# elliottower/gobblet-rl

Measured on AMD Instinct MI355X. Metric: env-steps/sec at 2^20 parallel boards, 1/2/4/8 MI355X; bit-exact mask/winner, higher is better.
Workload: dtype int8

## Files before the change

### gobblet-rl_amd/csrc/gobblet_hip.hip

```cpp
#include "gobblet_device.h"

#include <stdio.h>
#include <algorithm>
#include <type_traits>
#include <utility>
#include <stdlib.h>
#include <string.h>

#include "../../include/gobblet_hip.h"
#include "gobblet_diag.h"
#include "gobblet_knobs.h"

using namespace gbl;

namespace {

thread_local char g_err[256] = "";

int fail(int code, const char *msg)
{
    snprintf(g_err, sizeof g_err, "%s", msg);
    return code;
}

// ... 830 lines not shown
        }
        if (A.first_actions && t == 0) {
            action = given;
            if (SC)
                y = play_ply<false, PAIR>(p, row, mover, legal, action, A.illegal_mode, j);
            else
                y = play_ply<false, PAIR>(p, NoRow{}, mover, legal, action, A.illegal_mode, j);
        } else {
            if (SC)
                y = play_ply<true, PAIR>(p, row, mover, legal, action, A.illegal_mode, j);
            else
                y = play_ply<true, PAIR>(p, NoRow{}, mover, legal, action, A.illegal_mode, j);
        }
        GBL_PHASE_DEP(2, (uint32_t)y.winner + p.nz);
        dn = y.terminal ? 1 : 0;
        uint64_t legal_next = legal54(p, mover);
        if (y.terminal) {
            p = Planes{0u, 0u, 0u};
            mover = 0;
            legal_next = kLegalEmpty;
            if (SC) row.reset();
        }
        GBL_PHASE_DEP(3, p.nz);
        if (t) {
            if constexpr (OB) sub_store<kObs, kRowPolicy, BPS>(odst, vo, lane, obytes & ~15);
            if constexpr (MK) sub_store<kActions, kRowPolicy, BPS>(mdst, vm, lane, mbytes & ~15);
        }
        if constexpr (SC) {
            tcount = next_turn(tcount, y, 1);
            treset = treset || y.terminal;
            if (A.counters) {
                games += __popcll(__ballot(valid && j == 0 && y.terminal));
                w1 += __popcll(__ballot(valid && j == 0 && y.winner == 1));
                w2 += __popcll(__ballot(valid && j == 0 && y.winner == -1));
            }
            {
                const uint16_t rw = (uint16_t)((y.r0 & 0xFF) | ((y.r1 & 0xFF) << 8));
                if (sc_act) sc_act[at] = action;
                if (sc_rw) sc_rw[at] = rw;
                if (sc_b0) sc_b0[at] = (int8_t)(LPB == 1 ? y.winner : b0_is_mover ? mover : b0_is_winner ? y.winner : dn);
                if constexpr (LPB <= 2) {
                    if (sc_b1) sc_b1[at] = (int8_t)(LPB == 1 ? dn : y.winner);
                }
                if constexpr (LPB == 1) {
                    if (sc_b2) sc_b2[at] = (int8_t)mover;
                }
                at += A.ply_stride;
            }
        }
        GBL_PHASE(4);
        if constexpr (OB) {
            sub_obs_zero<BPS>(obs_img, lane);
            wave_lds_fence();
            obs_scatter_part<LPB>(reinterpret_cast<uint8_t *>(obs_img) + bq * kObs, p, mover, j);
            wave_lds_fence();
            odst = obs_at;
            obs_at += obs_step;
            sub_fetch<kObs, BPS>(obs_img, lane, vo);
            if (!full) sub_tail(odst, obs_img, lane, obytes);
            wave_lds_fence();
        }
        GBL_PHASE(5);
        legal = legal_next;
        GBL_PHASE_DEP(6, (uint32_t)legal);
        if constexpr (MK) {
            mask_row_part<LPB>(reinterpret_cast<uint8_t *>(mask_img) + bq * kActions, legal, j);
            wave_lds_fence();
            mdst = mask_at;
            mask_at += mask_step;
            sub_fetch<kActions, BPS>(mask_img, lane, vm);
            if (!full) sub_tail(mdst, mask_img, lane, mbytes);
            wave_lds_fence();
        }
        GBL_PHASE(7);
    }
    GBL_PHASE(7);
    GBL_PHASE_FLUSH(wave_index());
    if (plies) {
        if constexpr (OB) sub_store<kObs, kRowPolicy, BPS>(odst, vo, lane, obytes & ~15);
        if constexpr (MK) sub_store<kActions, kRowPolicy, BPS>(mdst, vm, lane, mbytes & ~15);
    }
    if constexpr (SC) {
        wave_lds_fence();
        sub_out<kCells, kStorePlain, BPS>(A.state + sub * (BPS * kCells), img, lane, rows);
        if (valid && j == 0) {
            A.to_move[b] = (int8_t)mover;
            A.done[b] = (int8_t)dn;
            if (A.turn) A.turn[b] = treset ? tcount : A.turn[b] + tcount;
        }
        if (A.counters && lane == 0) tally_flush(A.counters, sub >> SH, rows, plies, games, w1, w2);
    }
}

template <bool WITH_MASK, bool WITH_OBS, bool DEV_PLY, bool HAND>
__global__ __launch_bounds__(64 * (1 + (WITH_MASK ? 1 : 0) + (WITH_OBS ? 1 : 0))) void k_collect3(
    int8_t *__restrict__ state, int8_t *__restrict__ to_move, int64_t n, int64_t ntiles, uint64_t seed, uint64_t env_base,
    const uint32_t *__restrict__ ply_dev, uint32_t ply0, uint32_t plies, int8_t *__restrict__ done, int64_t ply_stride,
    int64_t tile_stride, int32_t *__restrict__ actions_t, int8_t *__restrict__ winner_t, int8_t *__restrict__ reward_t,
    int8_t *__restrict__ done_t, int8_t *__restrict__ to_move_t, int8_t *__restrict__ mask_t, int8_t *__restrict__ obs_t,
    int illegal_mode, int64_t *__restrict__ counters, int32_t *__restrict__ turn, const int32_t *__restrict__ first_actions,
    int8_t *__restrict__ first_status)
{
    constexpr int WAVES = 1 + (WITH_MASK ? 1 : 0) + (WITH_OBS ? 1 : 0);
    __shared__ uint32_t s_state[image_words<kCells>()];
    __shared__ uint32_t s_obs[WITH_OBS ? image_words<kObs>() : 4];
    __shared__ uint32_t s_mask[WITH_MASK ? image_words<kActions>() : 4];
    __shared__ uint4 s_hand[2][kTile];
    using LegalSlot = typename std::conditional<HAND, uint4, uint2>::type;
    __shared__ LegalSlot s_legal[2][kTile];
    if (DEV_PLY) ply0 += *ply_dev;
    const int role = WAVES > 1 ? wave_index() : 0;
    const int lane = (int)(threadIdx.x & 63u);
    const int64_t tile = (int64_t)blockIdx.x;
    if (tile >= ntiles) return;
    const int64_t left = n - tile * kTile;
    const int rows = left < kTile ? (int)left : kTile;
    const bool valid = lane < rows, full = rows == kTile;
    const int64_t b = tile * kTile + lane;
    constexpr int kPolicy = kStoreStreamDrop;
    const int64_t cell0 = tile * tile_stride;
    constexpr bool hand_scalars = HAND && WAVES > 1;
    if (role != 0) {
        const bool is_mask = WITH_MASK && role == 1;
        SubVecs<WITH_MASK ? sub_vectors<kActions, kTile>() : 0> vm{};
        SubVecs<WITH_OBS ? sub_vectors<kObs, kTile>() : 0> vo{};
        int8_t *dst = nullptr;
        int8_t *row_at = is_mask ? mask_t + cell0 * kActions : obs_t + cell0 * kObs;
        const int64_t row_step = ply_stride * (is_mask ? kActions : kObs);
        int64_t scell = cell0 + lane;
        for (uint32_t t = 0; t < plies; ++t) {
            pair_barrier();
            if constexpr (hand_scalars) {
                if (role == 1) {
                    const uint4 sc = s_legal[t & 1u][lane];
                    if (valid) {
                        if (actions_t) actions_t[scell] = (int32_t)sc.z;
                        if (winner_t) winner_t[scell] = (int8_t)(sc.w & 0xFFu);
                        if (reward_t) reinterpret_cast<uint16_t *>(reward_t)[scell] = (uint16_t)((sc.w >> 8) & 0xFFFFu);
                        if (done_t) done_t[scell] = (int8_t)((sc.w >> 24) & 1u);
                        if (to_move_t) to_move_t[scell] = (int8_t)((sc.w >> 25) & 1u);
                    }
                    scell += ply_stride;
                }
            }
            if (t) {
                if constexpr (WITH_MASK) {
                    if (is_mask) sub_store<kActions, kPolicy, kTile>(dst, vm, lane, (rows * kActions) & ~15);
                }
                if constexpr (WITH_OBS) {
                    if (!is_mask) sub_store<kObs, kPolicy, kTile>(dst, vo, lane, (rows * kObs) & ~15);
                }
            }
            if constexpr (WITH_MASK) {
                if (is_mask) {
                    const LegalSlot lg = s_legal[t & 1u][lane];
                    mask_row_part<1>(reinterpret_cast<uint8_t *>(s_mask) + lane * kActions, ((uint64_t)lg.y << 32) | lg.x, 0);
                    wave_lds_fence();
                    dst = row_at;
                    sub_fetch<kActions, kTile>(s_mask, lane, vm);
                    if (!full) sub_tail(dst, s_mask, lane, rows * kActions);
                    wave_lds_fence();
                }
            }
            if constexpr (WITH_OBS) {
                if (!is_mask) {
                    const uint4 h = s_hand[t & 1u][lane];
                    sub_obs_zero<kTile>(s_obs, lane);
                    wave_lds_fence();
                    obs_scatter_row(reinterpret_cast<uint8_t *>(s_obs) + lane * kObs, Planes{h.x, h.y, h.z}, (int)h.w);
                    wave_lds_fence();
                    dst = row_at;
                    sub_fetch<kObs, kTile>(s_obs, lane, vo);
                    if (!full) sub_tail(dst, s_obs, lane, rows * kObs);
                    wave_lds_fence();
                }
            }
            row_at += row_step;
        }
        if (plies) {
            if constexpr (WITH_MASK) {
                if (is_mask) sub_store<kActions, kPolicy, kTile>(dst, vm, lane, (rows * kActions) & ~15);
            }
            if constexpr (WITH_OBS) {
                if (!is_mask) sub_store<kObs, kPolicy, kTile>(dst, vo, lane, (rows * kObs) & ~15);
            }
        }
        return;
    }
    Lane L;
    L.tile = tile; L.lane = lane; L.rows = rows; L.valid = valid; L.b = b;
    int mover = to_move[valid ? b : n - 1];
    int given = first_actions ? first_actions[valid ? b : n - 1] : 0;
    uint32_t r[7];
    Draw4 block{{0u, 0u, 0u, 0u}};
    load_state(state, s_state, L, r, [&] { block = draw_block(seed, env_base + (uint64_t)b, ply0); });
    mover = valid && mover != 0;
    Planes p = planes_of(L, r);
    const ImageRow row{reinterpret_cast<uint8_t *>(s_state) + lane * kCells};
    uint32_t games = 0, w1 = 0, w2 = 0;
    Ply y{0, 0, 0, false, false};
    int dn = 0, tcount = 0;
    bool treset = false;
    uint64_t legal = legal54(p, mover);
    if (first_status && valid) first_status[b] = (int8_t)action_status_of(legal, given);
    int64_t cell = cell0;
    for (uint32_t t = 0; t < plies; ++t) {
        const uint32_t ply = ply0 + t;
        int action = pick54(legal, draw_word(block, ply));
        if (t + 1 < plies && ((ply + 1) & 3u) == 0) block = draw_block(seed, env_base + (uint64_t)b, ply + 1);
        if (first_actions && t == 0) {
            action = given;
            y = play_ply(p, row, mover, legal, action, illegal_mode);
        } else {
            y = play_ply<true>(p, row, mover, legal, action, illegal_mode);
        }
        dn = y.terminal ? 1 : 0;
        legal = legal54(p, mover);
        if (y.terminal) {
            p = Planes{0u, 0u, 0u};
            mover = 0;
            legal = kLegalEmpty;
            row.reset();
        }
        s_hand[t & 1u][lane] = uint4{p.nz, p.neg, p.odd, (uint32_t)mover};
        if constexpr (HAND)
            s_legal[t & 1u][lane] = uint4{(uint32_t)legal, (uint32_t)(legal >> 32), (uint32_t)action,
                                          ((uint32_t)y.winner & 0xFFu) | (((uint32_t)y.r0 & 0xFFu) << 8) | (((uint32_t)y.r1 & 0xFFu) << 16) |
                                              ((uint32_t)dn << 24) | ((uint32_t)mover << 25)};
        else
            s_legal[t & 1u][lane] = uint2{(uint32_t)legal, (uint32_t)(legal >> 32)};
        if (WAVES > 1) pair_barrier();
        tcount = next_turn(tcount, y, 1);
        treset = treset || y.terminal;
        if (counters) {
            games += __popcll(__ballot(valid && y.terminal));
            w1 += __popcll(__ballot(valid && y.winner == 1));
            w2 += __popcll(__ballot(valid && y.winner == -1));
        }
        if (!hand_scalars && valid) {
            const int64_t at = cell + lane;
            if (actions_t) actions_t[at] = action;
            if (winner_t) winner_t[at] = (int8_t)y.winner;
            if (reward_t) reinterpret_cast<uint16_t *>(reward_t)[at] = (uint16_t)((y.r0 & 0xFF) | ((y.r1 & 0xFF) << 8));
            if (done_t) done_t[at] = (int8_t)dn;
            if (to_move_t) to_move_t[at] = (int8_t)mover;
        }
        cell += ply_stride;
    }
    wave_lds_fence();
    tile_out<kCells>(state + tile * (kTile * kCells), s_state, lane, rows);
    if (valid) {
        to_move[b] = (int8_t)mover;
        done[b] = (int8_t)dn;
        if (turn) turn[b] = treset ? tcount : turn[b] + tcount;
    }
    if (counters && lane == 0) tally_flush(counters, tile, rows, plies, games, w1, w2);
}

template <bool WITH_MASK, bool WITH_OBS, int KO, bool MERGE>
constexpr int small_waves() { return 1 + ((WITH_MASK && !MERGE) ? 1 : 0) + (WITH_OBS ? KO : 0); }

template <bool WITH_MASK, bool WITH_OBS, bool DEV_PLY, int LA, int KO, bool MERGE>
__global__ __launch_bounds__((64 * small_waves<WITH_MASK, WITH_OBS, KO, MERGE>())) void k_collect_small(
    int8_t *__restrict__ state, int8_t *__restrict__ to_move, int64_t n, int64_t ngroups, uint64_t seed, uint64_t env_base,
    const uint32_t *__restrict__ ply_dev, uint32_t ply0, uint32_t plies, int8_t *__restrict__ done, int64_t ply_stride,
    int64_t tile_stride, int32_t *__restrict__ actions_t, int8_t *__restrict__ winner_t, int8_t *__restrict__ reward_t,
    int8_t *__restrict__ done_t, int8_t *__restrict__ to_move_t, int8_t *__restrict__ mask_t, int8_t *__restrict__ obs_t,
    int illegal_mode, int64_t *__restrict__ counters, int32_t *__restrict__ turn, const int32_t *__restrict__ first_actions,
    int8_t *__restrict__ first_status)
{
    static_assert(LA * KO <= 4 && (KO > 0 || MERGE), "at most four lanes per board");
    constexpr int WAVES = small_waves<WITH_MASK, WITH_OBS, KO, MERGE>(), NA = WAVES - (WITH_OBS ? KO : 0);
    constexpr int GB = kTile / LA, LO = LA * (KO ? KO : 1), OBB = kTile / LO;
    constexpr int kStateWords = GB * kCells / 4 + 4, kObsWords = OBB * kObs / 4 + 4, kMaskWords = GB * kActions / 4 + 4;
    __shared__ uint32_t s_state[WAVES][kStateWords];
    __shared__ uint32_t s_obs[WITH_OBS && KO ? KO : 1][WITH_OBS ? kObsWords : 4];
    __shared__ uint32_t s_mask[WITH_MASK ? kMaskWords : 4];
    __shared__ uint4 s_draw[LO > 1 ? WAVES : 1][LO > 1 ? 64 : 1];
    if (DEV_PLY) ply0 += *ply_dev;
    const int64_t group = (int64_t)blockIdx.x;
    if (group >= ngroups) return;
    const int wave = WAVES > 1 ? wave_index() : 0;
    const SmallArgs A{state, to_move, done, n, seed, env_base, ply0, plies, ply_stride, tile_stride, actions_t, winner_t, reward_t,
                      done_t, to_move_t, mask_t, obs_t, illegal_mode, counters, turn, first_actions, first_status};
    constexpr bool SYNC = WAVES > 1;
    if (wave == 0) {
        small_role<kRoleScalars | ((WITH_MASK && MERGE) ? kRoleMask : 0) | ((WITH_OBS && KO == 0) ? kRoleObs : 0), LA, SYNC>(
            A, s_state[0], s_mask, s_obs[0], reinterpret_cast<uint32_t *>(s_draw[0]), group);
        return;
    }
    if constexpr (WITH_MASK && !MERGE) {
        if (wave == 1) {
            small_role<kRoleMask, LA, SYNC>(A, s_state[1], s_mask, nullptr, reinterpret_cast<uint32_t *>(s_draw[LO > 1 ? 1 : 0]), group);
            return;
        }
    }
    if constexpr (WITH_OBS && KO > 0)
        small_role<kRoleObs, LO, SYNC>(A, s_state[wave], nullptr, s_obs[wave - NA], reinterpret_cast<uint32_t *>(s_draw[LO > 1 ? wave : 0]),
                                       group * KO + (wave - NA));
}

constexpr int kGroupBoards = 32, kGroupRing = 4;

template <bool WITH_OBS, bool DEV_PLY>
__global__ __launch_bounds__(64 * (WITH_OBS ? 4 : 2)) void k_collect5(
    int8_t *__restrict__ state, int8_t *__restrict__ to_move, int64_t n, int64_t ngroups, uint64_t seed, uint64_t env_base,
    const uint32_t *__restrict__ ply_dev, uint32_t ply0, uint32_t plies, int8_t *__restrict__ done, int64_t ply_stride,
    int64_t tile_stride, int32_t *__restrict__ actions_t, int8_t *__restrict__ winner_t, int8_t *__restrict__ reward_t,
    int8_t *__restrict__ done_t, int8_t *__restrict__ to_move_t, int8_t *__restrict__ mask_t, int8_t *__restrict__ obs_t,
    int illegal_mode, int64_t *__restrict__ counters, int32_t *__restrict__ turn, const int32_t *__restrict__ first_actions,
    int8_t *__restrict__ first_status)
{
    constexpr int GB = kGroupBoards, OBB = 16;
    static_assert(kGroupRing == 4, "slot = t & 7, one generator block per group of plies");
    __shared__ uint32_t s_state[GB * kCells / 4 + 4];
    __shared__ uint32_t s_mask[GB * kActions / 4 + 4];
    __shared__ uint32_t s_obs[WITH_OBS ? 2 : 1][WITH_OBS ? OBB * kObs / 4 + 4 : 4];
    __shared__ uint4 s_hand[2 * kGroupRing][GB];
    __shared__ uint4 s_legal[2 * kGroupRing][GB];
    __shared__ uint4 s_draw[4][GB];
    if (DEV_PLY) ply0 += *ply_dev;
    const int role = wave_index();
    const int lane = (int)(threadIdx.x & 63u);
    const int64_t group = (int64_t)blockIdx.x;
    if (group >= ngroups) return;
    const int64_t left = n - group * GB;
    const int rows = left < GB ? (int)left : GB;
    constexpr int kPolicy = kStoreStreamDrop;
    const int64_t cell0 = (group >> 1) * tile_stride + (group & 1) * GB;
    const uint32_t m0 = ply0 >> 2;
    const uint32_t groups_of_plies = (plies + kGroupRing - 1) / kGroupRing;
    if (role == 1) {
        const int bq = lane >> 1, j = lane & 1;
        const bool valid = bq < rows;
        const int64_t b = group * GB + bq;
        SubVecs<sub_vectors<kActions, GB>()> vm{};
        int8_t *dst = nullptr, *row_at = mask_t + cell0 * kActions;
        const int64_t row_step = ply_stride * kActions;
        const int mbytes = rows * kActions;
        int32_t *sc_act = nullptr;
        uint16_t *sc_rw = nullptr;
        int8_t *sc_b0 = nullptr, *sc_b1 = nullptr;
        if (valid) {
            const int64_t at0 = cell0 + bq;
            if (j == 0 && actions_t) sc_act = actions_t + at0;
            if (j == 1 && reward_t) sc_rw = reinterpret_cast<uint16_t *>(reward_t) + at0;
            int8_t *const arr = j == 0 ? to_move_t : done_t;
            if (arr) sc_b0 = arr + at0;
            if (j == 0 && winner_t) sc_b1 = winner_t + at0;
        }
        int64_t at = 0;
        uint32_t games = 0, w1 = 0, w2 = 0;
        int tcount = 0;
        bool treset = false;
        auto generate = [&](uint32_t m) {
            const Draw4 d = draw_block(seed, env_base + (uint64_t)b, m << 2);
            s_draw[m & 3u][bq] = uint4{d.w[0], d.w[1], d.w[2], d.w[3]};
        };
        generate(m0);
        generate(m0 + 1u);
        generate(m0 + 2u);
        pair_barrier();
        for (uint32_t g = 0; g < groups_of_plies; ++g) {
            pair_barrier();
            generate(m0 + g + 3u);
            const uint32_t t_end = (g + 1u) * kGroupRing < plies ? (g + 1u) * kGroupRing : plies;
#pragma nounroll
            for (uint32_t t = g * kGroupRing; t < t_end; ++t) {
                const uint4 sc = s_legal[t & (2u * kGroupRing - 1u)][bq];
                {
                    const uint32_t winner = sc.w & 0xFFu, dn = (sc.w >> 24) & 1u, mv = (sc.w >> 25) & 1u;
                    if (sc_act) sc_act[at] = (int32_t)sc.z;
                    if (sc_rw) sc_rw[at] = (uint16_t)((sc.w >> 8) & 0xFFFFu);
                    if (sc_b0) sc_b0[at] = (int8_t)(j == 0 ? mv : dn);
                    if (sc_b1) sc_b1[at] = (int8_t)winner;
                    at += ply_stride;
                    const bool terminal = dn != 0;
                    tcount = terminal ? 0 : tcount + (int)((sc.w >> 26) & 1u);
                    treset = treset || terminal;
                    if (counters) {
                        const int w = (int)(int8_t)winner;
                        games += __popcll(__ballot(valid && j == 0 && terminal));
                        w1 += __popcll(__ballot(valid && j == 0 && w == 1));
                        w2 += __popcll(__ballot(valid && j == 0 && w == -1));
                    }
                }
                if (t) sub_store<kActions, kPolicy, GB>(dst, vm, lane, mbytes & ~15);
                mask_row_part<2>(reinterpret_cast<uint8_t *>(s_mask) + bq * kActions, ((uint64_t)sc.y << 32) | sc.x, j);
                wave_lds_fence();
                dst = row_at;
                row_at += row_step;
                sub_fetch<kActions, GB>(s_mask, lane, vm);
                if (rows != GB) sub_tail(dst, s_mask, lane, mbytes);
                wave_lds_fence();
            }
        }
        if (plies) sub_store<kActions, kPolicy, GB>(dst, vm, lane, mbytes & ~15);
        if (valid && j == 0 && turn) turn[b] = treset ? tcount : turn[b] + tcount;
        if (counters && lane == 0) tally_flush(counters, group >> 1, rows, plies, games, w1, w2);
        return;
    }
    if (role >= 2) {
        if constexpr (WITH_OBS) {
            const int ow = role - 2, oq = lane >> 2, oj = lane & 3;
            const int orows_all = rows - ow * OBB, orows = orows_all < 0 ? 0 : orows_all > OBB ? OBB : orows_all;
            const int obytes = orows * kObs;
            uint32_t *const img = s_obs[ow];
            SubVecs<sub_vectors<kObs, OBB>()> vo{};
            int8_t *dst = nullptr, *row_at = obs_t + (cell0 + ow * OBB) * kObs;
            const int64_t row_step = ply_stride * kObs;
            pair_barrier();
            for (uint32_t g = 0; g < groups_of_plies; ++g) {
                pair_barrier();
                const uint32_t t_end = (g + 1u) * kGroupRing < plies ? (g + 1u) * kGroupRing : plies;
#pragma nounroll
                for (uint32_t t = g * kGroupRing; t < t_end; ++t) {
                    const uint4 h = s_hand[t & (2u * kGroupRing - 1u)][ow * OBB + oq];
                    if (t) sub_store<kObs, kPolicy, OBB>(dst, vo, lane, obytes & ~15);
                    sub_obs_zero<OBB>(img, lane);
                    wave_lds_fence();
                    obs_scatter_part<4>(reinterpret_cast<uint8_t *>(img) + oq * kObs, Planes{h.x, h.y, h.z}, (int)h.w, oj);
                    wave_lds_fence();
                    dst = row_at;
                    row_at += row_step;
                    sub_fetch<kObs, OBB>(img, lane, vo);
                    if (orows != OBB) sub_tail(dst, img, lane, obytes);
                    wave_lds_fence();
                }
            }
            if (plies) sub_store<kObs, kPolicy, OBB>(dst, vo, lane, obytes & ~15);
        }
        return;
    }
    const int bq = lane >> 1, j = lane & 1;
    const bool valid = bq < rows;
    const int64_t b = group * GB + bq, bs = valid ? b : n - 1;
    int mover = to_move[bs];
    int given = first_actions ? first_actions[bs] : 0;
    sub_in<kCells, GB>(state + group * (GB * kCells), s_state, lane, rows);
    wave_lds_fence();
    uint32_t r[7];
    row_load<kCells>(s_state, bq, r);
    r[6] &= 0x00FFFFFFu;
    mover = valid && mover != 0;
    Planes p = make_planes(r);
    p.nz = valid ? p.nz : 0u;
    int dn = 0;
    uint64_t legal = legal54(p, mover);
    if (first_status && valid && j == 0) first_status[b] = (int8_t)action_status_of(legal, given);
    pair_barrier();
    const uint32_t *const my_draws = reinterpret_cast<const uint32_t *>(&s_draw[0][bq]);
    uint32_t word = my_draws[(m0 & 3u) * (GB * 4) + (ply0 & 3u)];
    for (uint32_t t = 0; t < plies; ++t) {
        int action = pick54(legal, word);
        {
            const uint32_t nx = ply0 + t + 1u;
            word = my_draws[((nx >> 2) & 3u) * (GB * 4) + (nx & 3u)];
        }
        Ply y;
        if (first_actions && t == 0) {
            action = given;
            y = play_ply<false, true>(p, NoRow{}, mover, legal, action, illegal_mode, j);
        } else {
            y = play_ply<true, true>(p, NoRow{}, mover, legal, action, illegal_mode, j);
        }
        dn = y.terminal ? 1 : 0;
        legal = legal54(p, mover);
        if (y.terminal) {
            p = Planes{0u, 0u, 0u};
            mover = 0;
            legal = kLegalEmpty;
        }
        const uint32_t slot = t & (2u * kGroupRing - 1u);
        s_hand[slot][bq] = uint4{p.nz, p.neg, p.odd, (uint32_t)mover};
        s_legal[slot][bq] = uint4{(uint32_t)legal, (uint32_t)(legal >> 32), (uint32_t)action,
                                  ((uint32_t)y.winner & 0xFFu) | (((uint32_t)y.r0 & 0xFFu) << 8) | (((uint32_t)y.r1 & 0xFFu) << 16) |
                                      ((uint32_t)dn << 24) | ((uint32_t)mover << 25) | ((y.stepped ? 1u : 0u) << 26)};
        if ((t & (kGroupRing - 1u)) == kGroupRing - 1u || t + 1u == plies) pair_barrier();
    }
    planes_to_row(p, r);
    wave_lds_fence();
    if (j == 0) __builtin_memcpy(reinterpret_cast<uint8_t *>(s_state) + bq * kCells, r, kCells);
    wave_lds_fence();
    sub_out<kCells, kStorePlain, GB>(state + group * (GB * kCells), s_state, lane, rows);
    if (valid && j == 0) {
        to_move[b] = (int8_t)mover;
        done[b] = (int8_t)dn;
    }
}

template <bool WITH_A, bool WITH_B>
__global__ __launch_bounds__(64) void k_probe(int8_t *__restrict__ a, int8_t *__restrict__ b, int64_t ntiles, int plies)
{
    __shared__ uint32_t s_img[image_words<kObs>()];
    const int lane = threadIdx.x;
    const int64_t tile = blockIdx.x;
    if (tile >= ntiles) return;
    obs_image_zero(s_img, lane);
    wave_lds_fence();
    for (int t = 0; t < plies; ++t) {
        const int64_t cell = ((int64_t)t * ntiles + tile) * kTile;
        if (WITH_A) tile_out<kObs, kStoreStreamDrop>(a + cell * kObs, s_img, lane, kTile);
        if (WITH_B) tile_out<kActions, kStoreStreamDrop>(b + cell * kActions, s_img, lane, kTile);
    }
}

__global__ void k_counter_add(uint32_t *ctr, uint32_t by) { *ctr += by; }

__global__ __launch_bounds__(64) void k_sample(const int8_t *__restrict__ mask, int32_t *__restrict__ actions, int64_t n,
                                               int64_t ntiles, uint64_t seed, uint64_t env_base, uint32_t ply,
                                               const uint32_t *__restrict__ ply_dev)
{
    if (ply_dev) ply += *ply_dev;
    __shared__ uint32_t s_mask[image_words<kActions>()];
    Lane L;
    if (!lane_setup(L, n, ntiles)) return;
    uint32_t draw = 0;
    tile_in<kActions>(mask + L.tile * (kTile * kActions), s_mask, L.lane, L.rows,
                      [&] { draw = draw32(seed, env_base + (uint64_t)L.b, ply); });
    wave_lds_fence();
    uint32_t d[14];
    row_load<kActions>(s_mask, L.lane, d);
    if (!L.valid) return;
    actions[L.b] = pick54(mask_bits(d), draw);
}

__global__ __launch_bounds__(64) void k_decode_obs(const int8_t *__restrict__ obs, int8_t *__restrict__ state,
                                                   int8_t *__restrict__ to_move, int64_t n, int64_t ntiles)
{
    __shared__ uint32_t s_obs[image_words<kObs>()];
    __shared__ uint32_t s_state[image_words<kCells>()];
    Lane L;
    if (!lane_setup(L, n, ntiles)) return;
    tile_in<kObs>(obs + L.tile * (kTile * kObs), s_obs, L.lane, L.rows);
    wave_lds_fence();
    uint32_t d[30];
    row_load<kObs>(s_obs, L.lane, d);
    uint32_t r[7];
    int agent = decode_obs_row(d, r);
    row_stage<kCells>(s_state, L.lane, r);
    wave_lds_fence();
    tile_out<kCells>(state + L.tile * (kTile * kCells), s_state, L.lane, L.rows);
    if (L.valid) to_move[L.b] = (int8_t)agent;
}

__global__ __launch_bounds__(64) void k_validate(const int8_t *__restrict__ state, int8_t *__restrict__ flags, int64_t n,
                                                 int64_t ntiles)
{
    __shared__ uint32_t s_state[image_words<kCells>()];
    Lane L;
    if (!lane_setup(L, n, ntiles)) return;
    uint32_t r[7];
    load_state(state, s_state, L, r);
    if (!L.valid) return;
    flags[L.b] = (int8_t)validate_row(r);
}

__device__ __forceinline__ int uniform(int x) { return __builtin_amdgcn_readfirstlane(x); }

template <typename T>
__device__ __forceinline__ T wave_max(T x)
{
#pragma unroll
    for (int o = 32; o >= 1; o >>= 1) {
        const T other = __shfl_xor(x, o);
        x = other > x ? other : x;
    }
    return x;
}

__device__ __forceinline__ uint32_t wave_sum(uint32_t x)
{
#pragma unroll
    for (int o = 32; o >= 1; o >>= 1) x += (uint32_t)__shfl_xor((int)x, o);
    return x;
}

__device__ __forceinline__ Planes board_planes(const int8_t *__restrict__ state, int64_t b, uint32_t lane)
{
    const int v = lane < (uint32_t)kCells ? state[b * kCells + lane] : 0;
    return Planes{(uint32_t)__ballot(v != 0), (uint32_t)__ballot(v < 0), (uint32_t)__ballot(v & 1)};
}

__device__ __forceinline__ uint64_t board_candidates(const Planes &p, int mover, const int8_t *__restrict__ mask, int64_t b, uint32_t lane)
{
    uint64_t cand = legal54(p, mover);
    if (mask) cand &= (uint64_t)__ballot(lane < (uint32_t)kActions && mask[b * kActions + lane] != 0);
    return cand;
}

template <int W>
__global__ __launch_bounds__(64 * W) void k_playout(const int8_t *__restrict__ state, const int8_t *__restrict__ to_move,
                                                    const int8_t *__restrict__ mask, int32_t *__restrict__ wins_out,
                                                    int32_t *__restrict__ losses_out, int32_t *__restrict__ action_out,
                                                    int32_t *__restrict__ plies_out, int64_t n, uint64_t seed, uint64_t env_base,
                                                    uint32_t call, uint32_t K, uint64_t kinv, uint32_t max_plies)
{
    __shared__ uint32_t s_win[kActions], s_loss[kActions], s_plies;
    const uint32_t tid = threadIdx.x, lane = tid & 63u;
    for (int64_t b = blockIdx.x; b < n; b += gridDim.x) {
        for (uint32_t j = tid; j < (uint32_t)kActions; j += 64u * W) s_win[j] = s_loss[j] = 0u;
        if (tid == 0) s_plies = 0u;
        const Planes root = board_planes(state, b, lane);
        const int mover = to_move[b] != 0;
        const uint64_t cand = board_candidates(root, mover, mask, b, lane);
        const uint32_t total = (uint32_t)__popcll(cand) * K;
        __syncthreads();

        uint32_t item = tid, t = 0, plies = 0;
        Planes p = root;
        int side = mover, a = 0;
        uint64_t pid = 0;
        bool fresh = true;
        while (item < total) {
            if (fresh) {
                const uint32_t r = (uint32_t)(((uint64_t)item * kinv) >> 32);
                a = (int)kth_bit64(cand, r);
                pid = playout_id(env_base + (uint64_t)b, (uint32_t)a, item - r * K);
                p = root;
                side = mover;
                t = 0;
                fresh = false;
            }
            const Draw4 d = draw_block(seed, pid, playout_ply_index(call, t), kStreamPlayout);
#pragma unroll
            for (int u = 0; u < 4; ++u) {
                if (!fresh) {
                    const PlayoutEnd e = playout_end(playout_ply(p, side, t, a, d.w[u]), t, mover, max_plies);
                    ++t;
                    if (e.done) {
                        plies += e.plies;
                        if (e.outcome > 0) atomicAdd(&s_win[a], 1u);
                        if (e.outcome < 0) atomicAdd(&s_loss[a], 1u);
                        item += 64u * W;
                        fresh = true;
                    }
                }
            }
        }
        if (plies) atomicAdd(&s_plies, plies);
        __syncthreads();
        if (tid < 64u) {
            const bool in = lane < (uint32_t)kActions;
            const int w = in ? (int)s_win[lane] : 0, l = in ? (int)s_loss[lane] : 0;
            if (wins_out && in) wins_out[b * kActions + lane] = w;
            if (losses_out && in) losses_out[b * kActions + lane] = l;
            const uint32_t key = wave_max(in && ((cand >> lane) & 1ull) ? playout_key(w, l, (int)lane) : 0u);
            if (lane == 0) {
                if (action_out) action_out[b] = playout_action_of(key);
                if (plies_out) plies_out[b] = (int32_t)s_plies;
            }
        }
        __syncthreads();
    }
}

int playout_waves(int64_t n, int playouts)
{
    int w = 1;
    while (w < 8 && n * (2 * w) <= 16384 && 64 * (2 * w) * 4 <= 30 * playouts) w *= 2;
    return w;
}

struct TreeChild {
    uint32_t c, n, w, l;
    __device__ __forceinline__ bool mine() const { return c != 0u; }
    __device__ __forceinline__ uint32_t visits() const { return c ? n : 0u; }
};

__device__ __forceinline__ TreeChild tree_lane_child(const TreeNode *nodes, uint32_t first, uint32_t lane)
{
    TreeChild r{0u, 1u, 0u, 0u};
    for (uint32_t c = first; c;) {
        const TreeNode k = nodes[c];
        if (lane == tree_action(k)) r = TreeChild{c, k.n, tree_wins(k), tree_losses(k)};
        c = (uint32_t)__builtin_amdgcn_readfirstlane((int)k.sibling);
    }
    return r;
}

template <int W>
__device__ __forceinline__ void tree_iterations(TreeNode *const nodes, uint32_t (&s_sum)[2][2], const Planes &root, const int mover,
                                                const uint64_t cand, const uint64_t g, const uint64_t seed, const uint32_t call,
                                                const uint32_t iterations, const uint32_t P, const uint32_t max_plies,
                                                const uint32_t explore, const uint32_t tid, const uint32_t lane, uint32_t &count,
                                                uint32_t &plies_total)
{
    for (uint32_t i = 0; cand && i < iterations; ++i) {
        uint32_t v = 0, term;
        Planes p = root;
        int side = mover;
        uint64_t cd = cand, untried = 0;
        for (;;) {
            const TreeNode nv = nodes[v];
            term = tree_term(nv);
            if (term) break;
            const TreeChild my = tree_lane_child(nodes, nv.child, lane);
            untried = cd & ~(uint64_t)__ballot(my.mine());
            if (untried) break;
            const uint32_t key = wave_max(my.mine() ? tree_order_key(tree_key(my.w, my.l, my.n, P, nv.n, explore), lane) : 0u);
            const uint32_t a = (uint32_t)__builtin_amdgcn_readfirstlane((int)(63u - (key & 63u)));
            v = (uint32_t)__builtin_amdgcn_readlane((int)my.c, (int)a);
            move_planes(p, side, a);
            side ^= 1;
            cd = legal54(p, side);
        }
        const bool grow = term == kTreeOpen;
        uint32_t a_new = 0;
        if (grow) a_new = tree_expand_move(p, side, untried, draw32(seed, tree_pid(g, i, 0), playout_ply_index(call, 0), kStreamTree), term);
        uint32_t wl = 0, pl = 0;
        if (term == kTreeOpen) {
            uint32_t j = tid, t = 0;
            Planes q = p;
            int s = side;
            uint64_t pid = 0;
            bool fresh = true;
            while (j < P) {
                if (fresh) {
                    pid = tree_pid(g, i, j);
                    q = p;
                    s = side;
                    t = 0;
                    fresh = false;
                }
                const Draw4 d = draw_block(seed, pid, playout_ply_index(call, t), kStreamTree);
#pragma unroll
                for (int u = 0; u < 4; ++u) {
                    if (!fresh) {
                        const PlayoutEnd e = tree_playout_ply(q, s, side, t, d.w[u], max_plies);
                        ++t;
                        if (e.done) {
                            pl += e.plies;
                            wl += e.outcome > 0 ? 1u : (e.outcome < 0 ? 1u << 16 : 0u);
                            j += 64u * W;
                            fresh = true;
                        }
                    }
                }
            }
            wl = wave_sum(wl);
            pl = wave_sum(pl);
            if (W > 1 && lane == 0) {
                atomicAdd(&s_sum[i & 1u][0], wl);
                atomicAdd(&s_sum[i & 1u][1], pl);
            }
        }
        __syncthreads();
        if (W > 1 && term == kTreeOpen) {
            wl = s_sum[i & 1u][0];
            pl = s_sum[i & 1u][1];
        }
        if (term != kTreeOpen) wl = tree_decided(term, P);
        plies_total += pl;
        if (tid == 0) {
            if (W > 1) s_sum[(i & 1u) ^ 1u][0] = s_sum[(i & 1u) ^ 1u][1] = 0u;
            uint32_t leaf = v;
            if (grow) tree_link(nodes, leaf = count, v, a_new, term);
            tree_backup(nodes, leaf, wl & 0xFFFFu, wl >> 16);
        }
        count += grow ? 1u : 0u;
        __syncthreads();
    }
}

__device__ __forceinline__ uint64_t tree_root_out(const TreeNode *nodes, uint32_t lane, int64_t b, int32_t *__restrict__ visits_out,
                                                  int32_t *__restrict__ wins_out, int32_t *__restrict__ losses_out)
{
    const TreeChild c = tree_lane_child(nodes, nodes[0].child, lane);
    if (lane < (uint32_t)kActions) {
        if (visits_out) visits_out[b * kActions + lane] = (int32_t)c.visits();
        if (wins_out) wins_out[b * kActions + lane] = (int32_t)c.w;
        if (losses_out) losses_out[b * kActions + lane] = (int32_t)c.l;
    }
    return wave_max(c.mine() ? tree_final_key(c.n, c.w, c.l, lane) : 0ull);
}

template <int W>
__global__ __launch_bounds__(64 * W) void k_tree(const int8_t *__restrict__ state, const int8_t *__restrict__ to_move,
                                                 const int8_t *__restrict__ mask, int32_t *__restrict__ visits_out,
                                                 int32_t *__restrict__ wins_out, int32_t *__restrict__ losses_out,
                                                 int32_t *__restrict__ action_out, int32_t *__restrict__ nodes_out,
// ... 3403 lines not shown
```

Measured before the change: 38.57 billion.

## Expand mask and obs bit-packed rows directly into byte vectors, unroll ply ring

Removes the byte-image LDS staging buffers for mask and observation. The vector store payloads are built directly from the 54-bit legal words and from per-row obs bit quads, using a multiply trick that expands bits into bytes. The per-ply loops are unrolled by ring group, with a compile-time specialization on the draw offset, and the scalar stores use unconditional pointer bumps. Ballot-based counters are replaced by per-lane sums reduced once at the end. Together these cut LDS round-trips and fences, at the cost of more ALU work per vector and a larger unrolled code body that may raise register pressure.

```diff
diff --git a/gobblet-rl_amd/csrc/gobblet_hip.hip b/gobblet-rl_amd/csrc/gobblet_hip.hip
--- a/gobblet-rl_amd/csrc/gobblet_hip.hip
+++ b/gobblet-rl_amd/csrc/gobblet_hip.hip
@@ -1156,6 +1156,81 @@
 
 constexpr int kGroupBoards = 32, kGroupRing = 4;
 
+template <uint32_t V>
+struct Const {
+    static constexpr uint32_t value = V;
+};
+
+__device__ __forceinline__ uint4 bits_to_bytes16(uint32_t bits)
+{
+    uint32_t d[4];
+#pragma unroll
+    for (int k = 0; k < 4; ++k) d[k] = __umul24((bits >> (4 * k)) & 0xFu, 0x00204081u) & 0x01010101u;
+    return uint4{d[0], d[1], d[2], d[3]};
+}
+
+struct BitVec {
+    uint32_t wa, sh, mask_a, wb, na;
+};
+
+template <int ROWB, int ROWS>
+__device__ __forceinline__ BitVec bit_vec(int vec)
+{
+    constexpr int NV = ROWS * ROWB / 16;
+    const uint32_t v = (uint32_t)(vec < NV ? vec : NV - 1), byte0 = 16u * v, a = byte0 / (uint32_t)ROWB, off = byte0 - a * (uint32_t)ROWB;
+    const uint32_t na = (uint32_t)ROWB - off < 16u ? (uint32_t)ROWB - off : 16u;
+    return BitVec{a * 4u + (off >> 5), off & 31u, (1u << na) - 1u, (a + 1u < (uint32_t)ROWS ? a + 1u : (uint32_t)ROWS - 1u) * 4u, na};
+}
+
+__device__ __forceinline__ uint4 bit_vec_bytes(const uint32_t *w, const BitVec &g)
+{
+    const uint32_t lo = w[g.wa], hi = w[g.wa + 1], next = w[g.wb];
+    const uint32_t a = (uint32_t)((((uint64_t)hi << 32) | lo) >> g.sh);
+    return bits_to_bytes16((a & g.mask_a) | (next << g.na));
+}
+
+template <int ROWB, int ROWS>
+__device__ __forceinline__ uint2 bit_byte_at(int i)
+{
+    const uint32_t c = (uint32_t)(i < ROWS * ROWB ? i : ROWS * ROWB - 1), a = c / (uint32_t)ROWB, off = c - a * (uint32_t)ROWB;
+    return uint2{a * 4u + (off >> 5), off & 31u};
+}
+
+__device__ __forceinline__ uint4 obs_bits_quad(const Planes &p, int observer, int j)
+{
+    const uint32_t pos = p.nz & ~p.neg, ngv = p.nz & p.neg;
+    const uint32_t own = observer ? ngv : pos, opp = observer ? pos : ngv;
+    const uint32_t oddsel = (j & 1) ? ~p.odd : p.odd;
+    const uint32_t ownsel = own & oddsel, oppsel = opp & oddsel;
+    uint64_t lo = 0, hi = 0;
+#pragma unroll
+    for (int i = 0; i < 3; ++i) {
+        const int ch = j + 4 * i;
+        const uint32_t side = ch >= 6 ? oppsel : ownsel;
+        const int k = (ch >= 6 ? ch - 6 : ch) >> 1;
+        const uint32_t grp = (side >> (9 * k)) & 0x1FFu;
+        const uint32_t idx = 13u * (uint32_t)__builtin_ctz(grp | 0x100u) + (uint32_t)ch;
+        const uint64_t bit = (uint64_t)(grp ? 1u : 0u) << (idx & 63u);
+        lo |= idx < 64u ? bit : 0ull;
+        hi |= idx < 64u ? 0ull : bit;
+    }
+    uint32_t w[4] = {(uint32_t)lo, (uint32_t)(lo >> 32), (uint32_t)hi, (uint32_t)(hi >> 32)};
+#pragma unroll
+    for (int k = 0; k < 4; ++k) {
+        w[k] |= (uint32_t)__builtin_amdgcn_update_dpp(0, (int)w[k], 0xB1, 0xF, 0xF, false);
+        w[k] |= (uint32_t)__builtin_amdgcn_update_dpp(0, (int)w[k], 0x4E, 0xF, 0xF, false);
+    }
+    const uint32_t om = observer ? ~0u : 0u;
+    return uint4{w[0] | (om & 0x02001000u), w[1] | (om & 0x00080040u), w[2] | (om & 0x04002001u), w[3] | (om & 0x00100080u)};
+}
+
+__device__ __forceinline__ uint32_t lanes_sum(uint32_t x)
+{
+#pragma unroll
+    for (int o = 32; o >= 1; o >>= 1) x += (uint32_t)__shfl_xor((int)x, o);
+    return x;
+}
+
 template <bool WITH_OBS, bool DEV_PLY>
 __global__ __launch_bounds__(64 * (WITH_OBS ? 4 : 2)) void k_collect5(
     int8_t *__restrict__ state, int8_t *__restrict__ to_move, int64_t n, int64_t ngroups, uint64_t seed, uint64_t env_base,
@@ -1168,8 +1243,7 @@
     constexpr int GB = kGroupBoards, OBB = 16;
     static_assert(kGroupRing == 4, "slot = t & 7, one generator block per group of plies");
     __shared__ uint32_t s_state[GB * kCells / 4 + 4];
-    __shared__ uint32_t s_mask[GB * kActions / 4 + 4];
-    __shared__ uint32_t s_obs[WITH_OBS ? 2 : 1][WITH_OBS ? OBB * kObs / 4 + 4 : 4];
+    __shared__ uint4 s_obits[WITH_OBS ? 2 : 1][OBB + 1];
     __shared__ uint4 s_hand[2 * kGroupRing][GB];
     __shared__ uint4 s_legal[2 * kGroupRing][GB];
     __shared__ uint4 s_draw[4][GB];
@@ -1183,7 +1257,6 @@
     constexpr int kPolicy = kStoreStreamDrop;
     const int64_t cell0 = (group >> 1) * tile_stride + (group & 1) * GB;
     const uint32_t m0 = ply0 >> 2;
-    const uint32_t groups_of_plies = (plies + kGroupRing - 1) / kGroupRing;
     if (role == 1) {
         const int bq = lane >> 1, j = lane & 1;
         const bool valid = bq < rows;
@@ -1192,18 +1265,20 @@
         int8_t *dst = nullptr, *row_at = mask_t + cell0 * kActions;
         const int64_t row_step = ply_stride * kActions;
         const int mbytes = rows * kActions;
-        int32_t *sc_act = nullptr;
-        uint16_t *sc_rw = nullptr;
-        int8_t *sc_b0 = nullptr, *sc_b1 = nullptr;
-        if (valid) {
-            const int64_t at0 = cell0 + bq;
-            if (j == 0 && actions_t) sc_act = actions_t + at0;
-            if (j == 1 && reward_t) sc_rw = reinterpret_cast<uint16_t *>(reward_t) + at0;
-            int8_t *const arr = j == 0 ? to_move_t : done_t;
-            if (arr) sc_b0 = arr + at0;
-            if (j == 0 && winner_t) sc_b1 = winner_t + at0;
-        }
-        int64_t at = 0;
+        const int mwhole = __builtin_amdgcn_readfirstlane(mbytes & ~15);
+        const bool ragged = rows != GB;
+        const BitVec mv0 = bit_vec<kActions, GB>(lane), mv1 = bit_vec<kActions, GB>(lane + 64);
+        const int tail_i = (mbytes & ~15) + lane;
+        const bool tail_on = tail_i < mbytes;
+        const uint2 tail_at = bit_byte_at<kActions, GB>(tail_i);
+        const int bqs = valid ? bq : rows - 1;
+        const bool all_scalars = actions_t && winner_t && reward_t && done_t && to_move_t;
+        const int64_t at0 = cell0 + bqs;
+        const bool on_act = j == 0 && actions_t, on_rw = j == 1 && reward_t, on_b0 = j == 0 ? to_move_t != nullptr : done_t != nullptr,
+                   on_b1 = j == 0 && winner_t;
+        int32_t *sc_act = actions_t + at0;
+        uint16_t *sc_rw = reinterpret_cast<uint16_t *>(reward_t) + at0;
+        int8_t *sc_b0 = (j == 0 ? to_move_t : done_t) + at0, *sc_b1 = winner_t + at0;
         uint32_t games = 0, w1 = 0, w2 = 0;
         int tcount = 0;
         bool treset = false;
@@ -1211,47 +1286,68 @@
             const Draw4 d = draw_block(seed, env_base + (uint64_t)b, m << 2);
             s_draw[m & 3u][bq] = uint4{d.w[0], d.w[1], d.w[2], d.w[3]};
         };
+        auto ring_group = [&](auto check, uint32_t g) __attribute__((always_inline)) {
+            constexpr bool CHECK = decltype(check)::value != 0;
+            pair_barrier();
+            generate(m0 + g + 3u);
+            const uint4 *const ring = s_legal[(g & 1u) * kGroupRing];
+#pragma unroll
+            for (int u = 0; u < kGroupRing; ++u) {
+                if (CHECK && g * kGroupRing + (uint32_t)u >= plies) break;
+                const uint4 *const slot = ring + u * GB;
+                const uint4 sc = slot[bqs];
+                {
+                    const uint32_t winner = sc.w & 0xFFu, dn = (sc.w >> 24) & 1u, mv = (sc.w >> 25) & 1u;
+                    if (all_scalars) {
+                        *sc_b0 = (int8_t)(j == 0 ? mv : dn);
+                        if (j == 0) {
+                            *sc_act = (int32_t)sc.z;
+                            *sc_b1 = (int8_t)winner;
+                        } else {
+                            *sc_rw = (uint16_t)((sc.w >> 8) & 0xFFFFu);
+                        }
+                    } else {
+                        if (on_act) *sc_act = (int32_t)sc.z;
+                        if (on_rw) *sc_rw = (uint16_t)((sc.w >> 8) & 0xFFFFu);
+                        if (on_b0) *sc_b0 = (int8_t)(j == 0 ? mv : dn);
+                        if (on_b1) *sc_b1 = (int8_t)winner;
+                    }
+                    sc_act += ply_stride;
+                    sc_rw += ply_stride;
+                    sc_b0 += ply_stride;
+                    sc_b1 += ply_stride;
+                    const bool terminal = dn != 0;
+                    tcount = terminal ? 0 : tcount + (int)((sc.w >> 26) & 1u);
+                    treset = treset || terminal;
+                    games += dn;
+                    w1 += winner == 1u ? 1u : 0u;
+                    w2 += winner == 0xFFu ? 1u : 0u;
+                }
+                if (g || u) sub_store<kActions, kPolicy, GB>(dst, vm, lane, mwhole);
+                const uint32_t *const w = reinterpret_cast<const uint32_t *>(slot);
+                vm.template at<0>() = bit_vec_bytes(w, mv0);
+                vm.template at<1>() = bit_vec_bytes(w, mv1);
+                dst = row_at;
+                row_at += row_step;
+                if (ragged && tail_on) dst[tail_i] = (int8_t)((w[tail_at.x] >> tail_at.y) & 1u);
+            }
+        };
         generate(m0);
         generate(m0 + 1u);
         generate(m0 + 2u);
         pair_barrier();
-        for (uint32_t g = 0; g < groups_of_plies; ++g) {
-            pair_barrier();
-            generate(m0 + g + 3u);
-            const uint32_t t_end = (g + 1u) * kGroupRing < plies ? (g + 1u) * kGroupRing : plies;
-#pragma nounroll
-            for (uint32_t t = g * kGroupRing; t < t_end; ++t) {
-                const uint4 sc = s_legal[t & (2u * kGroupRing - 1u)][bq];
-                {
-                    const uint32_t winner = sc.w & 0xFFu, dn = (sc.w >> 24) & 1u, mv = (sc.w >> 25) & 1u;
-                    if (sc_act) sc_act[at] = (int32_t)sc.z;
-                    if (sc_rw) sc_rw[at] = (uint16_t)((sc.w >> 8) & 0xFFFFu);
-                    if (sc_b0) sc_b0[at] = (int8_t)(j == 0 ? mv : dn);
-                    if (sc_b1) sc_b1[at] = (int8_t)winner;
-                    at += ply_stride;
-                    const bool terminal = dn != 0;
-                    tcount = terminal ? 0 : tcount + (int)((sc.w >> 26) & 1u);
-                    treset = treset || terminal;
-                    if (counters) {
-                        const int w = (int)(int8_t)winner;
-                        games += __popcll(__ballot(valid && j == 0 && terminal));
-                        w1 += __popcll(__ballot(valid && j == 0 && w == 1));
-                        w2 += __popcll(__ballot(valid && j == 0 && w == -1));
-                    }
-                }
-                if (t) sub_store<kActions, kPolicy, GB>(dst, vm, lane, mbytes & ~15);
-                mask_row_part<2>(reinterpret_cast<uint8_t *>(s_mask) + bq * kActions, ((uint64_t)sc.y << 32) | sc.x, j);
-                wave_lds_fence();
-                dst = row_at;
-                row_at += row_step;
-                sub_fetch<kActions, GB>(s_mask, lane, vm);
-                if (rows != GB) sub_tail(dst, s_mask, lane, mbytes);
-                wave_lds_fence();
-            }
-        }
-        if (plies) sub_store<kActions, kPolicy, GB>(dst, vm, lane, mbytes & ~15);
+        const uint32_t whole_groups = plies / kGroupRing;
+        for (uint32_t g = 0; g < whole_groups; ++g) ring_group(Const<0>{}, g);
+        if (plies % kGroupRing) ring_group(Const<1>{}, whole_groups);
+        if (plies) sub_store<kActions, kPolicy, GB>(dst, vm, lane, mwhole);
         if (valid && j == 0 && turn) turn[b] = treset ? tcount : turn[b] + tcount;
-        if (counters && lane == 0) tally_flush(counters, group >> 1, rows, plies, games, w1, w2);
+        if (counters) {
+            const bool mine = valid && j == 0;
+            games = lanes_sum(mine ? games : 0u);
+            w1 = lanes_sum(mine ? w1 : 0u);
+            w2 = lanes_sum(mine ? w2 : 0u);
+            if (lane == 0) tally_flush(counters, group >> 1, rows, plies, games, w1, w2);
+        }
         return;
     }
     if (role >= 2) {
@@ -1259,30 +1355,41 @@
             const int ow = role - 2, oq = lane >> 2, oj = lane & 3;
             const int orows_all = rows - ow * OBB, orows = orows_all < 0 ? 0 : orows_all > OBB ? OBB : orows_all;
             const int obytes = orows * kObs;
-            uint32_t *const img = s_obs[ow];
+            const int owhole = __builtin_amdgcn_readfirstlane(obytes & ~15);
+            const bool ragged = orows != OBB;
+            uint4 *const rows_bits = s_obits[ow];
+            const uint32_t *const w = reinterpret_cast<const uint32_t *>(rows_bits);
             SubVecs<sub_vectors<kObs, OBB>()> vo{};
             int8_t *dst = nullptr, *row_at = obs_t + (cell0 + ow * OBB) * kObs;
             const int64_t row_step = ply_stride * kObs;
-            pair_barrier();
-            for (uint32_t g = 0; g < groups_of_plies; ++g) {
+            const BitVec ov0 = bit_vec<kObs, OBB>(lane), ov1 = bit_vec<kObs, OBB>(lane + 64);
+            const int tail_i = (obytes & ~15) + lane;
+            const bool tail_on = tail_i < obytes;
+            const uint2 tail_at = bit_byte_at<kObs, OBB>(tail_i);
+            auto ring_group = [&](auto check, uint32_t g) __attribute__((always_inline)) {
+                constexpr bool CHECK = decltype(check)::value != 0;
                 pair_barrier();
-                const uint32_t t_end = (g + 1u) * kGroupRing < plies ? (g + 1u) * kGroupRing : plies;
-#pragma nounroll
-                for (uint32_t t = g * kGroupRing; t < t_end; ++t) {
-                    const uint4 h = s_hand[t & (2u * kGroupRing - 1u)][ow * OBB + oq];
-                    if (t) sub_store<kObs, kPolicy, OBB>(dst, vo, lane, obytes & ~15);
-                    sub_obs_zero<OBB>(img, lane);
+                const uint4 *const mine = &s_hand[(g & 1u) * kGroupRing][ow * OBB + oq];
+#pragma unroll
+                for (int u = 0; u < kGroupRing; ++u) {
+                    if (CHECK && g * kGroupRing + (uint32_t)u >= plies) break;
+                    const uint4 h = mine[u * GB];
+                    if (g || u) sub_store<kObs, kPolicy, OBB>(dst, vo, lane, owhole);
+                    rows_bits[oq] = obs_bits_quad(Planes{h.x, h.y, h.z}, (int)h.w, oj);
                     wave_lds_fence();
-                    obs_scatter_part<4>(reinterpret_cast<uint8_t *>(img) + oq * kObs, Planes{h.x, h.y, h.z}, (int)h.w, oj);
-                    wave_lds_fence();
+                    vo.template at<0>() = bit_vec_bytes(w, ov0);
+                    vo.template at<1>() = bit_vec_bytes(w, ov1);
                     dst = row_at;
                     row_at += row_step;
-                    sub_fetch<kObs, OBB>(img, lane, vo);
-                    if (orows != OBB) sub_tail(dst, img, lane, obytes);
+                    if (ragged && tail_on) dst[tail_i] = (int8_t)((w[tail_at.x] >> tail_at.y) & 1u);
                     wave_lds_fence();
                 }
-            }
-            if (plies) sub_store<kObs, kPolicy, OBB>(dst, vo, lane, obytes & ~15);
+            };
+            pair_barrier();
+            const uint32_t whole_groups = plies / kGroupRing;
+            for (uint32_t g = 0; g < whole_groups; ++g) ring_group(Const<0>{}, g);
+            if (plies % kGroupRing) ring_group(Const<1>{}, whole_groups);
+            if (plies) sub_store<kObs, kPolicy, OBB>(dst, vo, lane, owhole);
         }
         return;
     }
@@ -1303,34 +1410,52 @@
     uint64_t legal = legal54(p, mover);
     if (first_status && valid && j == 0) first_status[b] = (int8_t)action_status_of(legal, given);
     pair_barrier();
-    const uint32_t *const my_draws = reinterpret_cast<const uint32_t *>(&s_draw[0][bq]);
-    uint32_t word = my_draws[(m0 & 3u) * (GB * 4) + (ply0 & 3u)];
-    for (uint32_t t = 0; t < plies; ++t) {
-        int action = pick54(legal, word);
-        {
-            const uint32_t nx = ply0 + t + 1u;
-            word = my_draws[((nx >> 2) & 3u) * (GB * 4) + (nx & 3u)];
-        }
-        Ply y;
-        if (first_actions && t == 0) {
-            action = given;
-            y = play_ply<false, true>(p, NoRow{}, mover, legal, action, illegal_mode, j);
-        } else {
-            y = play_ply<true, true>(p, NoRow{}, mover, legal, action, illegal_mode, j);
-        }
-        dn = y.terminal ? 1 : 0;
-        legal = legal54(p, mover);
-        if (y.terminal) {
-            p = Planes{0u, 0u, 0u};
-            mover = 0;
-            legal = kLegalEmpty;
-        }
-        const uint32_t slot = t & (2u * kGroupRing - 1u);
-        s_hand[slot][bq] = uint4{p.nz, p.neg, p.odd, (uint32_t)mover};
-        s_legal[slot][bq] = uint4{(uint32_t)legal, (uint32_t)(legal >> 32), (uint32_t)action,
-                                  ((uint32_t)y.winner & 0xFFu) | (((uint32_t)y.r0 & 0xFFu) << 8) | (((uint32_t)y.r1 & 0xFFu) << 16) |
-                                      ((uint32_t)dn << 24) | ((uint32_t)mover << 25) | ((y.stepped ? 1u : 0u) << 26)};
-        if ((t & (kGroupRing - 1u)) == kGroupRing - 1u || t + 1u == plies) pair_barrier();
+    const uint4 *const my_blocks = &s_draw[0][bq];
+    auto play = [&](auto a_tag) __attribute__((always_inline)) {
+        constexpr uint32_t A = decltype(a_tag)::value;
+        uint32_t mb = m0 & 3u;
+        uint4 cur = my_blocks[mb * GB], nxt = cur;
+        auto ring_group = [&](auto check, uint32_t g) __attribute__((always_inline)) {
+            constexpr bool CHECK = decltype(check)::value != 0;
+            mb = (mb + 1u) & 3u;
+            nxt = my_blocks[mb * GB];
+            const uint32_t words[8] = {cur.x, cur.y, cur.z, cur.w, nxt.x, nxt.y, nxt.z, nxt.w};
+            uint4 *const hand = &s_hand[(g & 1u) * kGroupRing][bq], *const lgl = &s_legal[(g & 1u) * kGroupRing][bq];
+#pragma unroll
+            for (int u = 0; u < kGroupRing; ++u) {
+                if (CHECK && g * kGroupRing + (uint32_t)u >= plies) break;
+                int action = pick54(legal, words[A + u]);
+                Ply y;
+                if (u == 0 && g == 0 && first_actions) {
+                    action = given;
+                    y = play_ply<false, true>(p, NoRow{}, mover, legal, action, illegal_mode, j);
+                } else {
+                    y = play_ply<true, true>(p, NoRow{}, mover, legal, action, illegal_mode, j);
+                }
+                dn = y.terminal ? 1 : 0;
+                legal = legal54(p, mover);
+                if (y.terminal) {
+                    p = Planes{0u, 0u, 0u};
+                    mover = 0;
+                    legal = kLegalEmpty;
+                }
+                hand[u * GB] = uint4{p.nz, p.neg, p.odd, (uint32_t)mover};
+                lgl[u * GB] = uint4{(uint32_t)legal, (uint32_t)(legal >> 32), (uint32_t)action,
+                                    ((uint32_t)y.winner & 0xFFu) | (((uint32_t)y.r0 & 0xFFu) << 8) | (((uint32_t)y.r1 & 0xFFu) << 16) |
+                                        ((uint32_t)dn << 24) | ((uint32_t)mover << 25) | ((y.stepped ? 1u : 0u) << 26)};
+            }
+            cur = nxt;
+            pair_barrier();
+        };
+        const uint32_t whole_groups = plies / kGroupRing;
+        for (uint32_t g = 0; g < whole_groups; ++g) ring_group(Const<0>{}, g);
+        if (plies % kGroupRing) ring_group(Const<1>{}, whole_groups);
+    };
+    switch (ply0 & 3u) {
+    case 0: play(Const<0>{}); break;
+    case 1: play(Const<1>{}); break;
+    case 2: play(Const<2>{}); break;
+    default: play(Const<3>{}); break;
     }
     planes_to_row(p, r);
     wave_lds_fence();
```

Result: no change. 38.58 billion (median of 6 runs) (+0.0%).
